# tardis-sn/tardis

Measured on AMD Instinct MI355X. Metric: packets/sec, higher is better.
Workload: dtype f64; 1 GPU; BASELINE configs[2]: 100000000 packets/GPU/step, 20 shells, 500000 lines, macroatom, 0 v-packets, last-interaction tracking on; synthetic opacities (SURVEY 8d, heavy-tailed macro-atom blocks), packets from the device black-body source (T_inner = 10000 K); level_sizes=heavy, packets_per_gpu=100000000, n_shells=20, n_lines=500000, line_interaction_type=macroatom, n_vpackets=0, parallelism=single GPU

## Files before the change

include/tardis_mc.h:

```cpp
#ifndef TARDIS_MC_H
#define TARDIS_MC_H

#include <stdint.h>

#ifdef __cplusplus
extern "C" {
#endif

#define TARDIS_MC_ABI_VERSION 2

enum {
    TARDIS_MC_OK = 0,
    TARDIS_MC_ERR_INVALID_ARGUMENT = -1,
    TARDIS_MC_ERR_HIP = -2,
    TARDIS_MC_ERR_MONTECARLO = -3,
    TARDIS_MC_ERR_MACRO_ATOM = -4,
    TARDIS_MC_ERR_UNSUPPORTED = -5,
    TARDIS_MC_ERR_COMM = -6,
    TARDIS_MC_ERR_STATE = -7
};

enum { TARDIS_MC_LINE_SCATTER = 0, TARDIS_MC_LINE_DOWNBRANCH = 1, TARDIS_MC_LINE_MACROATOM = 2 };

typedef struct TardisMcConfig {
// ... 355 lines not shown
int tardis_mc_streamed_packets(TardisMcContext *ctx, int64_t *out_streamed, int64_t *out_resent);

int tardis_mc_run(TardisMcContext *ctx, const TardisMcPackets *packets, const TardisMcGeometry *geometry,
                  const TardisMcOpacity *opacity, const TardisMcConfig *config, TardisMcResult *result);

#define TARDIS_MC_UNIQUE_ID_BYTES 128
int tardis_mc_comm_get_unique_id(uint8_t out_id[TARDIS_MC_UNIQUE_ID_BYTES]);
int tardis_mc_comm_init(TardisMcContext *ctx, int rank, int world_size,
                        const uint8_t id[TARDIS_MC_UNIQUE_ID_BYTES]);
int tardis_mc_allreduce_estimators(TardisMcContext *ctx);
int tardis_mc_comm_check(TardisMcContext *ctx, int *out_ranks);

int tardis_mc_debug_eval(TardisMcContext *ctx, int op, const double *x, const double *y, double *out, int64_t n);
int tardis_mc_debug_nlte_solve(TardisMcContext *ctx, int64_t n, int64_t n_systems, const double *m, const double *b, double *x, int32_t *status);
int tardis_mc_debug_microbench(TardisMcContext *ctx, int which, int64_t n_doubles, int iters, int blocks, double *out_ms);

#ifdef __cplusplus
}
#endif
#endif
```

tardis_amd/_lib.py:

```python
from __future__ import annotations

import ctypes as C
import os
import subprocess

from . import _abi

_HERE = os.path.dirname(os.path.abspath(__file__))
LIB_PATH = os.environ.get("TARDIS_MC_LIB") or os.path.join(_HERE, "libtardis_mc_hip.so")
_lib = None

_vp, _i, _ll = C.c_void_p, C.c_int, C.c_longlong
SYMBOLS = {
    "tardis_mc_abi_version": (_i, []),
    "tardis_mc_device_count": (_i, []),
    "tardis_mc_create": (_i, [_i, C.POINTER(_vp)]),
    "tardis_mc_destroy": (None, [_vp]),
    "tardis_mc_last_error": (C.c_char_p, [_vp]),
    "tardis_mc_set_option": (_i, [_vp, C.c_char_p, _ll]),
    "tardis_mc_set_geometry": (_i, [_vp, _vp]),
    "tardis_mc_set_opacity": (_i, [_vp, _vp]),
    "tardis_mc_set_config": (_i, [_vp, _vp]),
    "tardis_mc_set_packets": (_i, [_vp, _vp]),
    "tardis_mc_reset_estimators": (_i, [_vp]),
# ... 63 lines not shown
    "tardis_mc_set_nlte_collision_data": (_i, [_vp, _vp]),
    "tardis_mc_check_nlte_collision_data": (_i, [_vp, C.c_int64, _vp, C.c_double, C.c_int64, _vp]),
    "tardis_mc_get_nlte_collision_rates": (_i, [_vp, _vp, _vp]),
    "tardis_mc_get_event_log": (_i, [_vp, _vp]),
    "tardis_mc_get_vpacket_log": (_i, [_vp, _vp]),
    "tardis_mc_stream_results": (_i, [_vp, _vp]),
    "tardis_mc_streamed_packets": (_i, [_vp, C.POINTER(C.c_int64), C.POINTER(C.c_int64)]),
    "tardis_mc_run": (_i, [_vp] * 6),
    "tardis_mc_comm_get_unique_id": (_i, [_vp]),
    "tardis_mc_comm_init": (_i, [_vp, _i, _i, _vp]),
    "tardis_mc_allreduce_estimators": (_i, [_vp]),
    "tardis_mc_comm_check": (_i, [_vp, C.POINTER(_i)]),
    "tardis_mc_debug_eval": (_i, [_vp, _i, _vp, _vp, _vp, C.c_int64]),
    "tardis_mc_debug_nlte_solve": (_i, [_vp, C.c_int64, C.c_int64, _vp, _vp, _vp, _vp]),
    "tardis_mc_debug_microbench": (_i, [_vp, _i, C.c_int64, _i, _i, C.POINTER(C.c_double)]),
}


class EngineUnavailable(RuntimeError):
    """The HIP engine cannot be used (library not built, or no GPU)."""


def build(force: bool = False) -> str:
    cmd = ["make", "-C", os.path.join(_HERE, "csrc")] + (["-B"] if force else [])
    r = subprocess.run(cmd, capture_output=True, text=True)
    if r.returncode != 0:
        raise RuntimeError("building libtardis_mc_hip.so failed:\n" + r.stdout + r.stderr)
    return LIB_PATH


# ... 21 lines not shown
```

tardis_amd/csrc/mc_device.hpp:

```cpp
#pragma once
#include <hip/hip_runtime.h>
#include <stdint.h>
#include "mc_math.hpp"

namespace mc {

constexpr double C_LIGHT = 2.99792458e10;
constexpr double CLOSE_LINE_THRESHOLD = 1e-14;
constexpr double MISS_DISTANCE = 1e99;

enum : int { IT_BOUNDARY = 1, IT_LINE = 2, IT_ESCATTERING = 4 };
enum : int { ST_IN_PROCESS = 0, ST_EMITTED = 1, ST_REABSORBED = 2 };
enum : int { ERR_MONTECARLO = -3, ERR_MACRO_ATOM = -4, ERR_UNSUPPORTED = -5 };

constexpr int MT_N = 624;

template <bool WIDE> struct RowOffset { typedef unsigned type; };
template <> struct RowOffset<true> { typedef unsigned long long type; };
template <bool WIDE> using row_t = typename RowOffset<WIDE>::type;
template <bool WIDE> __host__ __device__ __forceinline__ row_t<WIDE> row_of(int shell, int len) { return (row_t<WIDE>)(unsigned)shell * (row_t<WIDE>)(unsigned)len; }

struct __attribute__((aligned(8))) LineVisitRecord {
    double c_e, c_jb;
    unsigned idx0;
// ... 96 lines not shown
    int n_shells, n_lines, n_trans;
    int line_interaction_type, disable_line_scattering, debug_flags, n_est_copies;
    double t_exp, sigma_thomson;
    double tc, rcp_tc;
    const double *r_inner, *r_outer, *nu_line, *tau_t, *n_e, *prob_t;
    const int2 *line_block;
    const int4 *trans_rec;
    const double *cum_t, *trans_nu;
    const unsigned short *cum16;
    const struct WalkRec *rec16;
    const int2 *quad_info;
    unsigned cum16_stride;
    const unsigned *hot_sec;
    const int2 *blk_tab;
    unsigned hot_stride;
    double *jblue_t, *edot_t;
    long long est_copy_stride;
    unsigned long long *next_packet;
    long long n_vpackets;
    double survival_probability, tau_russian, spawn_start, spawn_end, grid0, grid_last, delta_nu;
    double *vhist;
    const int *bucket_first;
    int bucket_shift, bucket_n;
    long long bucket_kmin;
    const double *tau_pfx, *tau_rowsum;
    const double *nt_t;
    unsigned nt_stride;
};

struct Packet {
// ... 215 lines not shown
```

tardis_amd/csrc/propagate_plan.hpp:

```cpp
#pragma once

#include "../../include/tardis_mc.h"

namespace plan {

constexpr int DBG_WALK_LANE_FP64 = 128;
constexpr int DBG_WALK_GROUP_FP64 = 8192;
constexpr int DBG_LONG_INSTANTIATIONS = 1048576;
constexpr int DBG_NO_SCREENING = 33554432;
constexpr int DBG_SKIP_FALLBACK = 536870912;
constexpr int DBG_WAVE_COUNTERS = 1 | 2 | 4 | 16 | 32 | 16384 | 32768 | 65536 | 131072 | 524288 | 2097152 | 4194304 | 8388608 | 16777216 | 134217728 | 268435456;
constexpr int DBG_FP64_WALKS = DBG_WALK_LANE_FP64 | DBG_WALK_GROUP_FP64;
constexpr int DBG_WAVE_CROSS_CHECK = DBG_FP64_WALKS | DBG_LONG_INSTANTIATIONS | DBG_WAVE_COUNTERS;

struct PlanInput {
    int n_shells, n_lines, n_trans;
    long long n_packets;
    long long number_of_vpackets;
    double survival_probability;
    int enable_full_relativity, line_interaction_type;
    bool lines_sorted, prob_negative, have_walk_tables;
    int variant, table_offsets, vpacket_screening;
    long long vpk_wave_min_packets;
    bool track_full;
    int debug_flags;
    bool pfx_valid, pfx_negative;
// ... 95 lines not shown
```

tardis_amd/csrc/propagate_wave.hpp:

```cpp
#pragma once
#include "mc_device.hpp"
#include "propagate_group.hpp"
#include "estimator_log.hpp"
#include "walk_tables.hpp"
#include "event_log.hpp"
#include "mt_generation.hpp"
#include "sweep_skip.hpp"

namespace mc {

constexpr int WV_STATE_STRIDE = 624;
constexpr int WV_RING = 8, WV_RING_VPK = 16;
enum : int { WS_NEED_PACKET = 0, WS_NEED_TRACE = 1, WS_SWEEP = 2, WS_DONE = 3, WS_WALK = 4, WS_VOLLEY = 5, WS_VCARRY = 6 };
constexpr int RES_PENDING = -1;
constexpr int WV_DBG_FLAGS = 1 | 2 | 4 | 16 | 32 | 16384 | 32768 | 65536 | 131072 | 524288 | 2097152 | 4194304 | 8388608 | 16777216 | 134217728 | 268435456;
constexpr int WV_RESERVE = 32;

struct WaveShared {
    double nu[64], rcp_nu[64], comov_nu[64], chi[64], rcp_chi[64], tau_event[64], d_cont0[64];
    double d_boundary[64];
    int res_info[64], res_line[64];
    unsigned rng_a[64], rng_b[64];
    int cursor[64], rowfast[64];
    int queue[64];
};
constexpr size_t WAVE_SHARED_LS_BYTES = sizeof(WaveShared) - 3 * 64 * sizeof(int);
static_assert(offsetof(WaveShared, queue) + sizeof(int) * 64 == sizeof(WaveShared) && offsetof(WaveShared, cursor) + 3 * 64 * sizeof(int) == sizeof(WaveShared),
              "cursor | rowfast | queue are the last 768 bytes: the lane-sweep instantiations leave them out, the pooled volleys' item list lies over them");
struct WaveSharedFull {
    double r[64], mu[64];
// ... 76 lines not shown
    LaneSave *save;
    WaveSave *wsave;
    int resume;
    int drain_split;
    unsigned *suspended;
    VolleyRequest *vq_req;
    unsigned *vq_items;
    unsigned *vq_count;
    int log_continue;
    int log_gen;
    double *vq_jsave;
    int rng_complete;
    int sweep_skip;
    unsigned sk_ct_off, sk_pn_off;
    double sk_margin;
};

__global__ void __launch_bounds__(64) late_list_kernel(const LaneSave *__restrict__ save, const WaveSave *__restrict__ wsave, int waves, long long first, long long end,
                                                       unsigned *__restrict__ late, unsigned *__restrict__ late_count, unsigned capacity)
{
    const int w = blockIdx.x, lane = threadIdx.x;
    if (w >= waves) return;
    const WaveSave ws = wsave[w];
    if (ws.done) return;
    const LaneSave &v = save[(size_t)w * 64 + lane];
    const bool live = v.state != WS_NEED_PACKET && v.state != WS_DONE && (long long)v.pkt >= first && (long long)v.pkt < end;
    const long long r0 = ws.res_next > first ? ws.res_next : first, r1 = ws.res_end < end ? ws.res_end : end;
    const int n_res = r1 > r0 ? (int)(r1 - r0) : 0;
    const unsigned long long lm = __ballot(live);
    const unsigned n_live = (unsigned)__popcll(lm);
// ... 583 lines not shown
    int ev_chunk = -1;
    unsigned ev_used = 0;
    bool ev_row = false;
    int ev_type = 0, ev_shell = 0, ev_after = 0, ev_absorb = -1, ev_emit = -1;
    double ev_bnu = 0.0, ev_bmu = 0.0, ev_be = 0.0;
    bool exhausted = false;
    long long res_next = 0, res_end = 0;
    int q_head = 0, q_tail = 0;
    unsigned log_used = 0;
    int log_chunk = -1;
    bool logged_any = false;
    unsigned long long visits = 0;
    constexpr bool DBG = XWALK;
    unsigned dbg_rounds = 0;
    unsigned long long dbg_vsteps = 0, dbg_vbusy = 0;
    unsigned dbg_walk = 0;
    bool s_active = false, s_fast = false;
    int s_line = 0;
    row_t<WIDE> s_row = 0;
    double s_tau = 0.0, s_tau_event = 0.0, s_kp = 0.0, s_xb = 0.0;
    int2 pre_blk = make_int2(0, 0);

    auto draw = [&]() {
        const double v = ring[r_head * 64 + lane];
        r_head = (r_head + 1) & (RING - 1);
        --r_cnt;
        ++draws;
        return v;
    };
    auto refill = [&](unsigned long long need, uint32_t *seeded_states) {
// ... 295 lines not shown
                    emit = p.next_line_id;
                    if (P.line_interaction_type != 0) {
                        const int2 blk = LS ? pre_blk : gload(P.line_block + (unsigned)p.next_line_id);
                        mb0 = blk.x; mb1 = blk.y;
                        in_macro = true;
                    }
                }
            }
        }
        TMC_SEC(1)
        if (P.cum16) {
            const int walk_cut = (DBG && (H.debug_flags & 16777216)) ? H.walk_min_active : (H.walk_min_active * __popcll(__ballot(state != WS_DONE))) >> 6;
            bool redo = false;
            double event = 0.0;
            if (resumed && mb1 >= 0 && (mb1 & WALK_REDO)) { redo = true; mb1 &= ~WALK_REDO; event = sh.tau_event[lane]; }
            for (int round = 0;; ++round) {
                const unsigned long long walking = __ballot(in_macro);
                if (!walking) break;
                if ((!VPK || !LS) && round > 0 && __popcll(walking) <= walk_cut && __ballot(!in_macro && state != WS_DONE)) break;
                refill(__ballot(in_macro && !redo && r_cnt < 1), seeded_states);
                unsigned x = 0;
                if (in_macro) {
                    if (!redo) event = draw();
                    x = (unsigned)(event * 65536.0);
                }
                const bool hot = in_macro && mb1 < 0, cold = in_macro && mb1 >= 0;
                int q_lo = 0, q_hi = cold ? (mb1 + 7) >> 3 : 0;
                const MC_G unsigned short *__restrict__ blk = glob(P.cum16) + ((size_t)p.shell * P.cum16_stride + (unsigned)(cold ? mb0 : 0));
                if (DBG && (H.debug_flags & 16384)) dbg_walk += (unsigned)__popcll(__ballot(cold && mb1 > 8 * WALK_WINDOW_QUADS));
                while (__ballot(cold && mb1 > 8 * WALK_WINDOW_QUADS && q_hi - q_lo > WALK_WINDOW_QUADS - 1)) {
                    if (cold && mb1 > 8 * WALK_WINDOW_QUADS && q_hi - q_lo > WALK_WINDOW_QUADS - 1) {
                        const int qm = q_lo + ((q_hi - q_lo) >> 1);
                        const unsigned v = blk[8 * qm + 7];
                        if (v < x) q_lo = qm + 1; else q_hi = qm;
                    }
                }
                int sel = -1;
                bool exact = false;
                int nxt = 0;
                unsigned nxt_arg = 0;
                if (in_macro) {
                    const int nq = hot ? 4 : min(WALK_WINDOW_QUADS, ((mb1 + 7) >> 3) - q_lo);
                    typedef unsigned u4v __attribute__((ext_vector_type(4)));
                    const MC_G u4v *__restrict__ wp = hot ? reinterpret_cast<const MC_G u4v *>(glob(P.hot_sec) + ((size_t)p.shell * (size_t)P.hot_stride + (size_t)(unsigned)mb0 * 16))
                                                          : reinterpret_cast<const MC_G u4v *>(blk + 8 * q_lo);
                    uint4 w0 = make_uint4(0, 0, 0, 0), w1 = w0, w2 = w0, w3 = w0;
                    if (nq > 0) { const u4v t = wp[0]; w0 = make_uint4(t.x, t.y, t.z, t.w); }
                    if (nq > 1) { const u4v t = wp[1]; w1 = make_uint4(t.x, t.y, t.z, t.w); }
                    if (nq > 2) { const u4v t = wp[2]; w2 = make_uint4(t.x, t.y, t.z, t.w); }
                    if (nq > 3) { const u4v t = wp[3]; w3 = make_uint4(t.x, t.y, t.z, t.w); }
                    if (hot) {
                        const unsigned lo2[3] = {w0.x, w0.y, w0.z}, hi2[3] = {w0.w, w1.x, w1.y}, k2[3] = {w3.x, w3.y, w3.z};
                        const unsigned dw[HOT_ENTRIES] = {w1.z, w1.w, w2.x, w2.y, w2.z, w2.w};
                        bool hit = false;
                        unsigned d = 0, k16 = 0;
#pragma unroll
                        for (int e = 0; e < HOT_ENTRIES; ++e) {
                            const unsigned sh16 = 16u * (unsigned)(e & 1);
                            const unsigned l = (lo2[e >> 1] >> sh16) & 0xffffu, h = (hi2[e >> 1] >> sh16) & 0xffffu;
                            if (x >= l && x < h) { hit = true; d = dw[e]; k16 = (k2[e >> 1] >> sh16) & 0xffffu; }
                        }
                        if (hit) {
                            macro += k16 + 1u;
                            if (d & WALK_EMIT) { emit = (int)(d & 0x7fffffffu); in_macro = false; nxt = 3; }
                            else if (d & WALK_HOT_DEST) mb0 = (int)(d & 0x3fffffffu);
                            else { nxt = 2; nxt_arg = d; }
                        } else { redo = true; nxt = 2; nxt_arg = (unsigned)mb0; }
                    } else {
                        const unsigned xx = x | (x << 16);
                        unsigned less = 0, gt = 0;
                        if (nq > 0) walk_count_quad(w0, xx, less, gt);
                        if (nq > 1) walk_count_quad(w1, xx, less, gt);
                        if (nq > 2) walk_count_quad(w2, xx, less, gt);
                        if (nq > 3) walk_count_quad(w3, xx, less, gt);
                        const int n_less = (int)((less & 0xffffu) + (less >> 16)), n_gt = (int)((gt & 0xffffu) + (gt >> 16));
                        int k = 8 * q_lo + n_less;
                        if (8 * nq - n_gt - n_less > 0) {
                            exact = true;
                            const MC_G double *__restrict__ cum = glob(P.cum_t) + (size_t)p.shell * (size_t)P.n_trans;
                            for (; k < mb1; ++k) {
                                const unsigned v = blk[k];
                                if (v > x) break;
                                const int2 qi = gload(P.quad_info + ((unsigned)(mb0 + k) >> 3));
                                if (cum[(unsigned)(qi.x + (k & 7))] > event) break;
                            }
                        }
                        if (k < mb1) sel = k;
                        macro += (unsigned)(sel >= 0 ? sel + 1 : mb1);
                        redo = false;
                        if (sel < 0) { err = ERR_MACRO_ATOM; in_macro = false; }
                        else nxt = 1;
                    }
                }
                if (DBG && (H.debug_flags & 32768)) dbg_walk += (unsigned)__popcll(__ballot(exact));
                if (DBG && (H.debug_flags & 65536)) dbg_walk += (unsigned)__popcll(__ballot(hot && !redo));
                if (DBG && (H.debug_flags & 131072)) dbg_walk += (unsigned)__popcll(__ballot(hot && redo));
                if (nxt == 1) {
                    const WalkRec rec = gload(P.rec16 + (unsigned)(mb0 + sel));
                    if (rec.b & WALK_EMIT) {
                        emit = (int)rec.a;
                        emit_nu_walk = rec.nu;
                        in_macro = false;
                        if (rec.b & WALK_UNSUPPORTED) err = ERR_UNSUPPORTED;
                    } else { mb0 = (int)rec.a; mb1 = (rec.b & WALK_HOT) ? -1 : (int)rec.b; }
                } else if (nxt == 2) {
                    const int2 bt = gload(P.blk_tab + nxt_arg);
                    mb0 = bt.x; mb1 = bt.y;
                } else if (nxt == 3)
                    emit_nu_walk = (NT != 0 && emit < L - 1) ? glob(P.nt_t)[2u * ((unsigned)p.shell * P.nt_stride + (unsigned)emit)]
                                                             : glob(P.nu_line)[(unsigned)emit];
            }
// ... 867 lines not shown
        }
        if (!keep) {
            if (cn[0]) gatomic_add_u64(&C->counters[0], cn[0]);
            if (cn[1]) gatomic_add_u64(&C->counters[1], cn[1]);
            if (cn[2]) gatomic_add_u64(&C->counters[2], cn[2]);
            if (cn[3]) gatomic_add_u64(&C->counters[5], cn[3]);
            if (VPK) {
                if (cn[4]) gatomic_add_u64(&C->counters[3], cn[4]);
                if (cn[5]) gatomic_add_u64(&C->counters[4], cn[5]);
                if (cn[6]) gatomic_add_u64(&C->counters[7], cn[6]);
            }
        }
        if (H.debug_flags & 16) gatomic_add_u64(&C->counters[7], (unsigned long long)dbg_rounds);
        if (VPK && (H.debug_flags & 134217728)) gatomic_add_u64(&C->counters[7], dbg_vbusy);
        if (VPK && (H.debug_flags & 268435456)) gatomic_add_u64(&C->counters[7], dbg_vsteps);
        if (H.debug_flags & (16384 | 32768 | 65536 | 131072)) gatomic_add_u64(&C->counters[7], (unsigned long long)dbg_walk);
        if (H.debug_flags & 2097152) gatomic_add_u64(&C->counters[7], dbg_drain_t0 ? wall_clock64() - dbg_drain_t0 : 0ull);
        if (H.debug_flags & 4194304) gatomic_add_u64(&C->counters[7], (unsigned long long)dbg_drain_passes);
        if (H.debug_flags & 8388608) gatomic_add_u64(&C->counters[7], (unsigned long long)dbg_drain_lanes);
        if (H.debug_flags & 32) gatomic_add_u64(&C->counters[7], (unsigned long long)dbg_passes);
#ifdef TMC_SECTION_TIMERS
        if (H.debug_flags & 64) {
            unsigned long long tsel = 0;
#pragma unroll
            for (int i = 0; i < 8; ++i) if (((H.debug_flags >> 8) & 7) == i) tsel = sec_t[i];
            gatomic_add_u64(&C->counters[7], tsel);
        }
#endif
    }
}

// ... 131 lines not shown
```

tardis_amd/csrc/tardis_mc_hip.hip:

```cpp
#include <hip/hip_runtime.h>
#include <dlfcn.h>

#include <algorithm>
#include <chrono>
#include <cstdarg>
#include <cstdio>
#include <cmath>
#include <cstring>
#include <functional>
#include <numeric>
#include <atomic>
#include <mutex>
#include <string>
#include <vector>

#include "../../include/tardis_mc.h"
#include "mc_device.hpp"
#include "propagate_lane.hpp"
#include "event_log.hpp"
#include "propagate_group.hpp"
#include "estimator_log.hpp"
#include "estimator_partition.hpp"
#include "propagate_wave.hpp"
#include "packet_source.hpp"
// ... 155 lines not shown
        long long bucket_kmin = 0;
        bool lines_sorted = true;
        bool prob_negative = false;
        std::vector<int> h_idx[5];
        std::vector<double> h_nu;
        bool h_macro = false;
        void release() { release_buffers(nu_line, tau_t, n_e, prob_t, cum_t, trans_nu, line2level, block_edge, ttype, dest, tline, line_block, trans_rec, bucket_first); }
    } ot;
    struct WalkTables {
        DevBuf cum16, rec16, quad_info, line_block_c;
        DevBuf hot_sec, hot_mass, hot_flag, blk_tab;
        bool have_hot = false;
        long long n_hot_blocks = 0;
        int walk_hot = -1;
        int walk_hot_min_mass = 800, walk_hot_min_mass_long = 400;
        unsigned cum16_stride = 0;
        bool have_walk_tables = false;
        int walk_sector_packing = 1;
        void release() { release_buffers(cum16, rec16, quad_info, line_block_c, hot_sec, hot_mass, hot_flag, blk_tab); }
    } wt;
    struct ScreeningTables {
        DevBuf tau_pfx, tau_rowsum, pfx_flag;
        bool pfx_valid = false, pfx_negative = false;
        int vpacket_screening = -1;
        void release() { release_buffers(tau_pfx, tau_rowsum, pfx_flag); }
    } sc;
    struct SweepTable {
        int sweep_table = -1;
        DevBuf nt_t;
        bool nt_valid = false, nt_negative = false;
// ... 37 lines not shown
    struct EventLog {
        bool track_full = false;
        long long evlog_capacity = 0;
        long long evlog_max_bytes = 16LL << 30;
        DevBuf ev_rows, ev_fill, ev_state, ev_counts, ev_offsets, ev_tiles, ev_cols;
        bool ev_valid = false;
        long long ev_packets = 0, ev_capacity = 0, ev_slots = 0;
        unsigned ev_chunk_rows = 128, ev_n_chunks = 0;
        void release() { release_buffers(ev_rows, ev_fill, ev_state, ev_counts, ev_offsets, ev_tiles, ev_cols); }
    } el;
    struct WaveResources {
        bool walk_min_active_user = false, ls_min_active_user = false;
        int walk_min_active = 8;
        int tracker_defer = 1, last_tracker_defer = -1;
        int rng_complete = 1;
        long long tracker_pack_max_lines = 0;
        int ls_min_active = 8, ls_max_steps = 1 << 30;
        int drain_split = 0;
        int log_tail_packets = 8;
        int log_tail_split = 1;
        int est_accumulate = 3;
        int est_pipeline = 1;
        DevBuf log_part;
        long long log_chunk_records = 0;
        long long log_capacity = 2500000000LL;
        bool log_capacity_user = false;
        hipStream_t stream2 = nullptr;
        hipEvent_t ev_join = nullptr;
        int pass_cus = 0, pass_cus_built = 0;
        hipStream_t stream_prop_m = nullptr, stream_pass_m = nullptr;
// ... 1307 lines not shown
    wc.vp_scratch = ctx->wv.vp_scratch.as<mc::VpResult>();
    wc.vp_park = (vpk && !E.vq_on && ctx->wv.vp_carry_min_active > 0) ? ctx->wv.vp_park.as<mc::VpPark>() : nullptr;
    wc.vp_carry_min_active = ctx->wv.vp_carry_min_active; wc.trk_defer = E.trk_defer;
    wc.save = E.may_suspend ? E.cur_save : nullptr;
    wc.wsave = E.may_suspend ? E.cur_wsave : nullptr;
    wc.resume = epoch > 0 ? 1 : 0;
    wc.drain_split = E.split_armed ? 64 : (E.compact_armed ? ctx->wv.drain_compact : 0);
    wc.suspended = ctx->wv.suspended_dev.as<unsigned>();
    wc.vq_req = E.vq_on ? ctx->wv.vq_req.as<mc::VolleyRequest>() : nullptr;
    wc.vq_items = E.vq_on ? ctx->wv.vq_items.as<unsigned>() : nullptr;
    wc.vq_count = vq ? ctx->wv.vq_count.as<unsigned>() : nullptr;
    wc.vq_jsave = vq ? ctx->wv.vq_jsave.as<double>() : nullptr;
    wc.log_continue = vq ? 1 : 0;
    wc.log_gen = E.log_gen;
    wc.rng_complete = ctx->wv.rng_complete;
    wc.sweep_skip = E.sweep_skip; wc.sk_ct_off = ctx->sw.sk_ct_off; wc.sk_pn_off = ctx->sw.sk_pn_off; wc.sk_margin = ctx->sw.sk_margin;
    HIP_TRY(ctx, store_value(E.st, wc_dev, wc));
    return TARDIS_MC_OK;
}

int launch_second_half(TardisMcContext *ctx, WaveCall &E, int epoch, int waves1, hipStream_t es, mc::WaveCold *wc_dev)
{
    const mc::WaveCold &wc = ctx->wv.wave_cold_host[epoch & 1];
    mc::WaveCold wc2 = wc;
    wc2.seeded_states = wc.seeded_states + (size_t)waves1 * 64 * mc::WV_STATE_STRIDE;
    if (wc.save) wc2.save = wc.save + (size_t)waves1 * 64;
    if (wc.wsave) wc2.wsave = wc.wsave + waves1;
    if (wc.vp_scratch) wc2.vp_scratch = wc.vp_scratch + (size_t)waves1 * 64 * mc::VP_ROUND;
    if (wc.vp_park) wc2.vp_park = wc.vp_park + (size_t)waves1 * 64;
    HIP_TRY(ctx, hipStreamWaitEvent(es, ctx->wv.ev_split[0], 0));
// ... 221 lines not shown
    const bool vpk = call.vpk, full = call.full, vq = call.plan.variant == 4;
    const int cus = call.cus;
    const long long n = ctx->pk.n_packets;
    const mc::DeviceProblem &F = ctx->problem_host;
    if (n >= (1LL << 31)) return fail(ctx, TARDIS_MC_ERR_INVALID_ARGUMENT, "more than 2^31 packets per propagate call");
    WaveChoice w{};
    int rc = choose_wave_kernel(ctx, call, P, w);
    if (rc) return rc;
    if (w.compact_walk) {
        P.cum16 = ctx->wt.cum16.as<unsigned short>(); P.rec16 = ctx->wt.rec16.as<mc::WalkRec>(); P.quad_info = ctx->wt.quad_info.as<int2>();
        P.cum16_stride = ctx->wt.cum16_stride;
        P.line_block = ctx->wt.line_block_c.as<int2>();
        P.hot_sec = ctx->wt.have_hot ? ctx->wt.hot_sec.as<unsigned>() : nullptr;
        P.blk_tab = ctx->wt.blk_tab.as<int2>();
        P.hot_stride = (unsigned)(16u * (unsigned)ctx->n_levels);
    }
    ctx->pg.progress_wave = true;
    const int n_xcd = 8;
    const bool cu_split = ctx->wv.pass_cus > 0 && !vq && ctx->wv.log_sets != 1 && cus == 32 * n_xcd && n >= 30000000LL;
    const int cus_prop = cu_split ? cus - n_xcd * ctx->wv.pass_cus : cus;
    const int waves = (int)std::max<long long>(1, std::min<long long>((n + 63) / 64, (long long)cus_prop * std::min(w.waves_per_cu, w.max_waves_per_cu) * (vq ? ctx->wv.vq_oversubscribe : 1)));
    if (ctx->el.track_full) {
        rc = setup_event_log(ctx, ctx->problem_host, 4LL * waves);
        if (rc) return rc;
    }
    if (ctx->wv.events_host && ctx->wv.ev_events && hipEventQuery(ctx->wv.ev_events) == hipSuccess && ctx->wv.events_host[1] > 0)
        ctx->wv.traces_per_packet = (double)ctx->wv.events_host[0] / (double)ctx->wv.events_host[1];
    if (1.1 * ctx->wv.traces_per_packet > ctx->wv.log_budget_per_packet) ctx->wv.log_budget_per_packet = 1.3 * ctx->wv.traces_per_packet;
    LogSizing s{};
    rc = size_line_log(ctx, call, w, n, waves, cu_split, s);
// ... 309 lines not shown
    else if (n == "blocks_per_cu") ctx->blocks_per_cu = std::max(1, (int)value);
    else if (n == "track_last_interaction") ctx->pk.track = value != 0;
    else if (n == "estimator_copies") { ctx->es.est_copies = std::max(1, std::min(8, (int)value)); ctx->es.est_valid = false; }
    else if (n == "vpacket_log_capacity") { ctx->vl.vlog_capacity = value; ctx->vl.vlog_capacity_user = value > 0; }
    else if (n == "track_full") ctx->el.track_full = value != 0;
    else if (n == "vpacket_last_interaction") ctx->vl.vlog_li = value != 0;
    else if (n == "event_log_capacity") ctx->el.evlog_capacity = std::max<long long>(0, value);
    else if (n == "event_log_max_bytes") ctx->el.evlog_max_bytes = std::max<long long>(1LL << 20, value);
    else if (n == "debug_flags") ctx->debug_flags = (int)value;
    else if (n == "drain_split") ctx->wv.drain_split = value ? 1 : 0;
    else if (n == "drain_compact") ctx->wv.drain_compact = (int)std::max<long long>(0, std::min<long long>(48, value));
    else if (n == "est_one_level") ctx->wv.est_one_level = value ? 1 : 0;
    else if (n == "drain_pack_lanes") ctx->wv.drain_pack_lanes = (int)std::max<long long>(1, std::min<long long>(64, value));
    else if (n == "walk_sector_packing") ctx->wt.walk_sector_packing = value ? 1 : 0;
    else if (n == "walk_hot") ctx->wt.walk_hot = value < 0 ? -1 : (value ? 1 : 0);
    else if (n == "walk_hot_min_mass") ctx->wt.walk_hot_min_mass = (int)std::max<long long>(0, std::min<long long>(value, 1001));
    else if (n == "walk_hot_min_mass_long") ctx->wt.walk_hot_min_mass_long = (int)std::max<long long>(0, std::min<long long>(value, 1001));
    else if (n == "vpacket_screening") ctx->sc.vpacket_screening = value < 0 ? -1 : (value ? 1 : 0);
    else if (n == "waves_per_simd") ctx->waves_per_simd = (int)value;
    else if (n == "lane_sweep_min_active") {
        ctx->wv.ls_min_active_user = value >= 0;
        ctx->wv.ls_min_active = value >= 0 ? (int)std::min<long long>(value, 63) : 8;
    }
    else if (n == "lane_sweep_max_steps") ctx->wv.ls_max_steps = (int)std::max<long long>(1, value);
    else if (n == "vq_oversubscribe") ctx->wv.vq_oversubscribe = (int)std::max<long long>(1, std::min<long long>(value, 64));
    else if (n == "vq_tracer_waves_per_simd") ctx->wv.vq_tracer_waves_per_simd = (int)std::max<long long>(1, std::min<long long>(value, 16));
    else if (n == "vq_min_items") ctx->wv.vq_min_items = value;
    else if (n == "vq_min_active") ctx->wv.vq_min_active = (int)std::max<long long>(0, std::min<long long>(value, 63));
    else if (n == "log_tail_split") ctx->wv.log_tail_split = value ? 1 : 0;
    else if (n == "est_pipeline") ctx->wv.est_pipeline = value ? 1 : 0;
// ... 5 lines not shown
    else if (n == "stream_min_packets") ctx->rs.min_packets = std::max<long long>(64, value);
    else if (n == "sweep_table") ctx->sw.sweep_table = (int)std::max<long long>(-1, std::min<long long>(value, 2));
    else if (n == "table_offsets") ctx->table_offsets = value < 0 ? -1 : (value ? 1 : 0);
    else if (n == "vpk_wide_registers") ctx->vpk_wide_registers = (int)std::max<long long>(0, std::min<long long>(value, 2));
    else if (n == "bucket_lines_permille") ctx->ot.bucket_lines_permille = (int)std::max<long long>(50, std::min<long long>(value, 16000));
    else if (n == "vp_carry_min_active") ctx->wv.vp_carry_min_active = (int)std::max<long long>(0, std::min<long long>(value, 63));
    else if (n == "est_accumulate") ctx->wv.est_accumulate = (int)std::max<long long>(0, std::min<long long>(value, 3));
    else if (n == "log_tail_packets") ctx->wv.log_tail_packets = (int)std::max<long long>(0, std::min<long long>(value, 1000));
    else if (n == "log_chunk_records") ctx->wv.log_chunk_records = value <= 0 ? 0 : std::max<long long>(256, std::min<long long>(value, 1 << 20));
    else if (n == "walk_min_active") {
        ctx->wv.walk_min_active_user = value >= -1;
        ctx->wv.walk_min_active = value >= -1 ? (int)std::min<long long>(value, 63) : 8;
    }
    else if (n == "tracker_defer") ctx->wv.tracker_defer = value ? 1 : 0;
    else if (n == "rng_complete") ctx->wv.rng_complete = value ? 1 : 0;
    else if (n == "sweep_skip") ctx->sw.sweep_skip = (int)std::max<long long>(-1, std::min<long long>(value, 1));
    else if (n == "tracker_pack_max_lines") ctx->wv.tracker_pack_max_lines = std::max<long long>(0, value);
    else if (n == "group_size") ctx->group_size = (value == 4 || value == 8 || value == 16) ? (int)value : 0;
    else if (n == "pipeline_chunks") {}
    else if (n == "log_capacity") { ctx->wv.log_capacity = std::max<long long>(0, value); ctx->wv.log_capacity_user = true; }
    else if (n == "log_sets") ctx->wv.log_sets = (value == 1 || value == 2) ? (int)value : 0;
    else if (n == "source_max_iterations") ctx->sf.max_iterations = std::max<long long>(1, value);
    else if (n == "chunk_packets") ctx->chunk_packets = std::max<long long>(1024, value);
    else if (n == "opacity_update_long_rows") ctx->ou.long_rows = value < 0 ? -1 : value;
    else if (n == "plasma_update_long_rows") ctx->pl.long_rows = value < 0 ? -1 : value;
    else if (n == "mean_opacity_long_bins") ctx->mo.long_bins = value < 0 ? -1 : value;
    else if (n == "plasma_max_iterations") ctx->pl.max_iterations = std::max<long long>(1, value);
    else if (n == "nlte_lds_levels") ctx->nl.lds_levels = value < 0 ? -1 : value;
    else if (n == "nlte_blocked_levels") ctx->nl.blocked_levels = value < 0 ? -1 : value;
    else return fail(ctx, TARDIS_MC_ERR_INVALID_ARGUMENT, "unknown option '%s'", name);
// ... 51 lines not shown
        long long tc = 0;
        for (size_t b = 0; b < n_levels; ++b) {
            const long long len = (edge[b + 1] - edge[b] + 7) / 8 * 8;
            if (ctx->wt.walk_sector_packing && len > 0) {
                const long long in_sector = tc & 31;
                if (in_sector != 0 && (len > 32 || in_sector + len > 32)) tc += 32 - in_sector;
            }
            c0[b] = tc;
            tc += len;
        }
        c0[n_levels] = tc;
        const long long n_quads = tc / 8;
        const unsigned long long stride = ((unsigned long long)tc + 31ull) / 32ull * 32ull + mc::WALK_SLACK;
        if (tc > 0 && stride * S < (1ull << 32) && tc < (1LL << 30)) {
            std::vector<unsigned char> hot(n_levels, 0);
            if (ctx->wt.walk_hot != 0 && n_levels < (size_t)mc::WALK_HOT) {
                const long long nb = (long long)n_levels * (long long)S;
                HIP_TRY(ctx, ctx->wt.hot_sec.ensure((size_t)nb * 64));
                HIP_TRY(ctx, ctx->wt.hot_mass.ensure((size_t)nb * sizeof(unsigned)));
                HIP_TRY(ctx, ctx->wt.hot_flag.ensure(n_levels));
                auto launch_hot = [&](const unsigned char *flags, unsigned *mass) {
                    hipLaunchKernelGGL(mc::walk_hot_kernel, dim3((unsigned)((nb + 255) / 256)), dim3(256), 0, ctx->stream, ctx->ot.cum_t.as<double>(),
                                       ctx->ot.block_edge.as<int>(), ctx->ot.ttype.as<int>(), ctx->ot.dest.as<int>(), ctx->ot.tline.as<int>(), flags,
                                       (int)n_levels, (long long)T, (int)S, ctx->wt.hot_sec.as<unsigned>(), mass);
                    return hipGetLastError();
                };
                HIP_TRY(ctx, launch_hot(nullptr, ctx->wt.hot_mass.as<unsigned>()));
                std::vector<unsigned> mass((size_t)nb);
                HIP_TRY(ctx, hipMemcpyAsync(mass.data(), ctx->wt.hot_mass.p, (size_t)nb * sizeof(unsigned), hipMemcpyDeviceToHost, ctx->stream));
                HIP_TRY(ctx, hipStreamSynchronize(ctx->stream));
                for (size_t b = 0; b < n_levels; ++b) {
                    const long long rows = edge[b + 1] - edge[b];
                    if (rows <= 0) continue;
                    double m = 0.0;
                    for (size_t sh = 0; sh < S; ++sh) m += (double)mass[sh * n_levels + b];
                    m /= 65536.0 * (double)S;
                    const double need = 1e-3 * (double)(rows > 8 * mc::WALK_WINDOW_QUADS ? ctx->wt.walk_hot_min_mass_long : ctx->wt.walk_hot_min_mass);
                    if (ctx->wt.walk_hot == 1 || m >= need) { hot[b] = 1; ctx->wt.n_hot_blocks += 1; }
                }
                if (ctx->wt.n_hot_blocks > 0) {
                    HIP_TRY(ctx, hipMemcpyAsync(ctx->wt.hot_flag.p, hot.data(), n_levels, hipMemcpyHostToDevice, ctx->stream));
                    hipLaunchKernelGGL(mc::walk_hot_flag_kernel, dim3((unsigned)((nb + 255) / 256)), dim3(256), 0, ctx->stream, ctx->wt.hot_flag.as<unsigned char>(), nb,
                                       ctx->wt.hot_sec.as<unsigned>());
                    HIP_TRY(ctx, hipGetLastError());
                    HIP_TRY(ctx, hipStreamSynchronize(ctx->stream));
                    ctx->wt.have_hot = true;
                } else {
                    ctx->wt.hot_sec.release();
                    ctx->wt.hot_flag.release();
                }
                ctx->wt.hot_mass.release();
            }
            {
                std::vector<int> bt(2 * n_levels);
                for (size_t b = 0; b < n_levels; ++b) {
                    bt[2 * b] = (int)c0[b];
                    bt[2 * b + 1] = (int)(edge[b + 1] - edge[b]);
                }
                if ((rc = upload(ctx, ctx->wt.blk_tab, bt.data(), bt.size()))) return rc;
                HIP_TRY(ctx, hipStreamSynchronize(ctx->stream));
            }
            std::vector<int> qi(2 * (size_t)n_quads, 0), lbc(2 * L, 0);
            std::vector<mc::WalkRec> r16((size_t)tc + 1, mc::WalkRec{0u, 0u, 0.0});
            for (size_t b = 0; b < n_levels; ++b) {
                const long long b0 = edge[b], b1 = edge[b + 1];
                for (long long q = c0[b] / 8, k = b0; k < b1; ++q, k += 8) { qi[2 * q] = (int)k; qi[2 * q + 1] = (int)(b1 - k); }
                for (long long k = b0; k < b1; ++k) {
                    const long long c = c0[b] + (k - b0);
                    const int64_t tt = ttype[k];
                    if (tt >= 0) {
                        const int64_t lvl = dest[k];
                        if (hot[lvl]) { r16[c].a = (unsigned)lvl; r16[c].b = mc::WALK_HOT; }
                        else {
                            r16[c].a = (unsigned)c0[lvl];
                            r16[c].b = (unsigned)(edge[lvl + 1] - edge[lvl]);
// ... 2898 lines not shown
    hipLaunchKernelGGL(comm_check_fill_kernel, dim3(1), dim3(64), 0, ctx->stream, cell.as<double>(), (double)(ctx->rank + 1));
    hipError_t e = hipGetLastError();
    int r = e == hipSuccess ? g_rccl.AllReduce(cell.p, cell.p, 1, 8, 0, ctx->comm, ctx->stream) : 0;
    double got = 0.0;
    if (e == hipSuccess && r == 0) e = hipMemcpyAsync(&got, cell.p, sizeof(double), hipMemcpyDeviceToHost, ctx->stream);
    if (e == hipSuccess && r == 0) e = hipStreamSynchronize(ctx->stream);
    HIP_TRY(ctx, e);
    if (r != 0) return fail(ctx, TARDIS_MC_ERR_COMM, "ncclAllReduce failed: %s", g_rccl.GetErrorString ? g_rccl.GetErrorString(r) : "?");
    const double want = 0.5 * (double)ctx->world * (double)(ctx->world + 1);
    if (got != want)
        return fail(ctx, TARDIS_MC_ERR_COMM, "communicator self-check: the sum of (rank + 1) over %d ranks came back as %.17g, not %.17g", ctx->world, got, want);
    *out_ranks = ctx->world;
    return TARDIS_MC_OK;
}

int tardis_mc_debug_eval(TardisMcContext *ctx, int op, const double *x, const double *y, double *out, int64_t n)
{
    if (!ctx || !x || !out || n <= 0) return TARDIS_MC_ERR_INVALID_ARGUMENT;
    HIP_TRY(ctx, hipSetDevice(ctx->device));
    if (op == 100) {
        const long long first = (long long)x[0], count = n / 8;
        if (n % 8 || first < 0 || first + count > ctx->pk.n_packets || !ctx->pk.li_rec.p || ctx->wv.last_tracker_defer < 0)
            return fail(ctx, TARDIS_MC_ERR_STATE, "debug_eval: no tracker records of a wave-kernel call for packets [%lld, %lld)", first, first + count);
        HIP_TRY(ctx, hipStreamSynchronize(ctx->stream));
        HIP_TRY(ctx, hipMemcpy(out, (const char *)ctx->pk.li_rec.p + (size_t)first * 64, (size_t)count * 64, hipMemcpyDeviceToHost));
        return TARDIS_MC_OK;
    }
    ScopedDevBuf dx, dy, dout, scratch;
    size_t nx = (op == 7) ? 1 : (size_t)n;
    HIP_TRY(ctx, dx.ensure(nx * 8));
// ... 87 lines not shown
```

tardis_amd/csrc/walk_tables.hpp:

```cpp
#pragma once
#include <hip/hip_runtime.h>
#include <stdint.h>

namespace mc {

constexpr unsigned WALK_EMIT = 0x80000000u, WALK_UNSUPPORTED = 0x40000000u;
constexpr unsigned WALK_HOT = 0x20000000u;
constexpr unsigned WALK_HOT_DEST = 0x40000000u;
constexpr int WALK_REDO = 0x40000000;
constexpr int HOT_ENTRIES = 6;
struct __attribute__((aligned(16))) WalkRec {
    unsigned a, b;
    double nu;
};
constexpr int WALK_WINDOW_QUADS = 4;
constexpr int WALK_SLACK = 8 * WALK_WINDOW_QUADS;

__global__ void __launch_bounds__(256) walk_cum16_kernel(const double *__restrict__ cum_t, const int2 *__restrict__ quad_info,
                                                          long long n_quads, long long n_trans, int n_shells, unsigned stride,
                                                          unsigned short *__restrict__ cum16)
{
    const long long i = (long long)blockIdx.x * blockDim.x + threadIdx.x;
    if (i >= n_quads * n_shells) return;
    const long long q = i % n_quads;
    const int s = (int)(i / n_quads);
    const int2 info = quad_info[q];
    const double *c = cum_t + (long long)s * n_trans + info.x;
    unsigned v[8];
#pragma unroll
    for (int k = 0; k < 8; ++k) {
        unsigned e = 0xffffu;
// ... 60 lines not shown
                    t0 = kk[e]; kk[e] = nk; nk = t0;
                }
        }
    }
    unsigned total = 0;
#pragma unroll
    for (int e = 0; e < HOT_ENTRIES; ++e) total += wd[e];
    uint4 *out = reinterpret_cast<uint4 *>(hot_sec + ((size_t)s * (size_t)n_blocks + (size_t)b) * 16);
    out[0] = make_uint4(lo[0] | (lo[1] << 16), lo[2] | (lo[3] << 16), lo[4] | (lo[5] << 16), hi[0] | (hi[1] << 16));
    out[1] = make_uint4(hi[2] | (hi[3] << 16), hi[4] | (hi[5] << 16), dw[0], dw[1]);
    out[2] = make_uint4(dw[2], dw[3], dw[4], dw[5]);
    out[3] = make_uint4(kk[0] | (kk[1] << 16), kk[2] | (kk[3] << 16), kk[4] | (kk[5] << 16), total);
    if (mass) mass[(size_t)s * (size_t)n_blocks + (size_t)b] = total;
}

__global__ void __launch_bounds__(256) walk_hot_flag_kernel(const unsigned char *__restrict__ hot_flag, long long n_records, unsigned *__restrict__ hot_sec)
{
    const long long i = (long long)blockIdx.x * blockDim.x + threadIdx.x;
    if (i >= n_records) return;
    unsigned *rec = hot_sec + (size_t)i * 16;
    const unsigned lo3[3] = {rec[0], rec[1], rec[2]}, hi3[3] = {rec[3], rec[4], rec[5]};
#pragma unroll
    for (int e = 0; e < HOT_ENTRIES; ++e) {
        const unsigned sh16 = 16u * (unsigned)(e & 1);
        const unsigned l = (lo3[e >> 1] >> sh16) & 0xffffu, h = (hi3[e >> 1] >> sh16) & 0xffffu;
        const unsigned d = rec[6 + e];
        if (h > l && !(d & WALK_EMIT) && hot_flag[d & 0x3fffffffu]) rec[6 + e] = d | WALK_HOT_DEST;
    }
}

typedef unsigned short walk_u16x2 __attribute__((ext_vector_type(2)));
__device__ __forceinline__ void walk_count(unsigned d, unsigned xx, unsigned &less, unsigned &gt)
{
    const walk_u16x2 dv = __builtin_bit_cast(walk_u16x2, d), xv = __builtin_bit_cast(walk_u16x2, xx);
    const walk_u16x2 one = {1, 1};
    walk_u16x2 l = __builtin_elementwise_sub_sat(xv, dv);
    walk_u16x2 g = __builtin_elementwise_sub_sat(dv, xv);
    l = __builtin_elementwise_min(l, one);
    g = __builtin_elementwise_min(g, one);
    less = __builtin_bit_cast(unsigned, (walk_u16x2)(__builtin_bit_cast(walk_u16x2, less) + l));
    gt = __builtin_bit_cast(unsigned, (walk_u16x2)(__builtin_bit_cast(walk_u16x2, gt) + g));
}
__device__ __forceinline__ void walk_count_quad(const uint4 &w, unsigned xx, unsigned &less, unsigned &gt)
// ... 6 lines not shown
```

Baseline: 43.23 million packets/s.

## Pack destination block offsets into hot walk records and add cold-batch walk rounds

```diff
diff --git a/include/tardis_mc.h b/include/tardis_mc.h
--- a/include/tardis_mc.h
+++ b/include/tardis_mc.h
@@ -393,6 +393,7 @@
 int tardis_mc_debug_eval(TardisMcContext *ctx, int op, const double *x, const double *y, double *out, int64_t n);
 int tardis_mc_debug_nlte_solve(TardisMcContext *ctx, int64_t n, int64_t n_systems, const double *m, const double *b, double *x, int32_t *status);
 int tardis_mc_debug_microbench(TardisMcContext *ctx, int which, int64_t n_doubles, int iters, int blocks, double *out_ms);
+int tardis_mc_debug_walk_pack(int64_t c0, int64_t rows, int q_bits, int own, int rows_cap, uint32_t *word, int64_t *c0_back, int64_t *rows_back);
 
 #ifdef __cplusplus
 }
diff --git a/tardis_amd/_lib.py b/tardis_amd/_lib.py
--- a/tardis_amd/_lib.py
+++ b/tardis_amd/_lib.py
@@ -101,6 +101,7 @@
     "tardis_mc_debug_eval": (_i, [_vp, _i, _vp, _vp, _vp, C.c_int64]),
     "tardis_mc_debug_nlte_solve": (_i, [_vp, C.c_int64, C.c_int64, _vp, _vp, _vp, _vp]),
     "tardis_mc_debug_microbench": (_i, [_vp, _i, C.c_int64, _i, _i, C.POINTER(C.c_double)]),
+    "tardis_mc_debug_walk_pack": (_i, [C.c_int64, C.c_int64, _i, _i, _i, C.POINTER(C.c_uint32), C.POINTER(C.c_int64), C.POINTER(C.c_int64)]),
 }
 
 
diff --git a/tardis_amd/csrc/mc_device.hpp b/tardis_amd/csrc/mc_device.hpp
--- a/tardis_amd/csrc/mc_device.hpp
+++ b/tardis_amd/csrc/mc_device.hpp
@@ -134,6 +134,7 @@
     const unsigned *hot_sec;
     const int2 *blk_tab;
     unsigned hot_stride;
+    int walk_q;
     double *jblue_t, *edot_t;
     long long est_copy_stride;
     unsigned long long *next_packet;
diff --git a/tardis_amd/csrc/propagate_plan.hpp b/tardis_amd/csrc/propagate_plan.hpp
--- a/tardis_amd/csrc/propagate_plan.hpp
+++ b/tardis_amd/csrc/propagate_plan.hpp
@@ -9,7 +9,7 @@
 constexpr int DBG_LONG_INSTANTIATIONS = 1048576;
 constexpr int DBG_NO_SCREENING = 33554432;
 constexpr int DBG_SKIP_FALLBACK = 536870912;
-constexpr int DBG_WAVE_COUNTERS = 1 | 2 | 4 | 16 | 32 | 16384 | 32768 | 65536 | 131072 | 524288 | 2097152 | 4194304 | 8388608 | 16777216 | 134217728 | 268435456;
+constexpr int DBG_WAVE_COUNTERS = 1 | 2 | 4 | 16 | 32 | 16384 | 32768 | 65536 | 131072 | 262144 | 524288 | 2097152 | 4194304 | 8388608 | 16777216 | 134217728 | 268435456;
 constexpr int DBG_FP64_WALKS = DBG_WALK_LANE_FP64 | DBG_WALK_GROUP_FP64;
 constexpr int DBG_WAVE_CROSS_CHECK = DBG_FP64_WALKS | DBG_LONG_INSTANTIATIONS | DBG_WAVE_COUNTERS;
 
diff --git a/tardis_amd/csrc/propagate_wave.hpp b/tardis_amd/csrc/propagate_wave.hpp
--- a/tardis_amd/csrc/propagate_wave.hpp
+++ b/tardis_amd/csrc/propagate_wave.hpp
@@ -13,7 +13,7 @@
 constexpr int WV_RING = 8, WV_RING_VPK = 16;
 enum : int { WS_NEED_PACKET = 0, WS_NEED_TRACE = 1, WS_SWEEP = 2, WS_DONE = 3, WS_WALK = 4, WS_VOLLEY = 5, WS_VCARRY = 6 };
 constexpr int RES_PENDING = -1;
-constexpr int WV_DBG_FLAGS = 1 | 2 | 4 | 16 | 32 | 16384 | 32768 | 65536 | 131072 | 524288 | 2097152 | 4194304 | 8388608 | 16777216 | 134217728 | 268435456;
+constexpr int WV_DBG_FLAGS = 1 | 2 | 4 | 16 | 32 | 16384 | 32768 | 65536 | 131072 | 262144 | 524288 | 2097152 | 4194304 | 8388608 | 16777216 | 134217728 | 268435456;
 constexpr int WV_RESERVE = 32;
 
 struct WaveShared {
@@ -120,6 +120,7 @@
     int sweep_skip;
     unsigned sk_ct_off, sk_pn_off;
     double sk_margin;
+    int walk_cold_batch;
 };
 
 __global__ void __launch_bounds__(64) late_list_kernel(const LaneSave *__restrict__ save, const WaveSave *__restrict__ wsave, int waves, long long first, long long end,
@@ -733,6 +734,7 @@
     constexpr bool DBG = XWALK;
     unsigned dbg_rounds = 0;
     unsigned long long dbg_vsteps = 0, dbg_vbusy = 0;
+    unsigned dbg_walk_hi = 0;
     unsigned dbg_walk = 0;
     bool s_active = false, s_fast = false;
     int s_line = 0;
@@ -1058,17 +1060,33 @@
             bool redo = false;
             double event = 0.0;
             if (resumed && mb1 >= 0 && (mb1 & WALK_REDO)) { redo = true; mb1 &= ~WALK_REDO; event = sh.tau_event[lane]; }
+            const int cold_k = (LS && !VPK) ? W->walk_cold_batch : 0;
+            unsigned long long moved = 0;
+            bool last_round = false;
             for (int round = 0;; ++round) {
                 const unsigned long long walking = __ballot(in_macro);
-                if (!walking) break;
-                if ((!VPK || !LS) && round > 0 && __popcll(walking) <= walk_cut && __ballot(!in_macro && state != WS_DONE)) break;
-                refill(__ballot(in_macro && !redo && r_cnt < 1), seeded_states);
+                if (!walking || last_round) break;
+                const bool cut = (!VPK || !LS) && round > 0 && __popcll(walking) <= walk_cut && __ballot(!in_macro && state != WS_DONE);
+                bool act = in_macro;
+                if (cold_k > 0) {
+                    if (cut) {
+                        if (!(walking & ~moved)) break;
+                        act = in_macro && !((moved >> lane) & 1ull);
+                        last_round = true;
+                    } else {
+                        const unsigned long long cold_w = __ballot(in_macro && mb1 >= 0);
+                        const bool cold_round = cold_w == walking || __popcll(cold_w) >= cold_k;
+                        act = in_macro && ((mb1 >= 0) == cold_round);
+                    }
+                    moved |= __ballot(act);
+                } else if (cut) break;
+                refill(__ballot(act && !redo && r_cnt < 1), seeded_states);
                 unsigned x = 0;
-                if (in_macro) {
+                if (act) {
                     if (!redo) event = draw();
                     x = (unsigned)(event * 65536.0);
                 }
-                const bool hot = in_macro && mb1 < 0, cold = in_macro && mb1 >= 0;
+                const bool hot = act && mb1 < 0, cold = act && mb1 >= 0;
                 int q_lo = 0, q_hi = cold ? (mb1 + 7) >> 3 : 0;
                 const MC_G unsigned short *__restrict__ blk = glob(P.cum16) + ((size_t)p.shell * P.cum16_stride + (unsigned)(cold ? mb0 : 0));
                 if (DBG && (H.debug_flags & 16384)) dbg_walk += (unsigned)__popcll(__ballot(cold && mb1 > 8 * WALK_WINDOW_QUADS));
@@ -1083,7 +1101,8 @@
                 bool exact = false;
                 int nxt = 0;
                 unsigned nxt_arg = 0;
-                if (in_macro) {
+                bool packed_dest = false;
+                if (act) {
                     const int nq = hot ? 4 : min(WALK_WINDOW_QUADS, ((mb1 + 7) >> 3) - q_lo);
                     typedef unsigned u4v __attribute__((ext_vector_type(4)));
                     const MC_G u4v *__restrict__ wp = hot ? reinterpret_cast<const MC_G u4v *>(glob(P.hot_sec) + ((size_t)p.shell * (size_t)P.hot_stride + (size_t)(unsigned)mb0 * 16))
@@ -1108,8 +1127,13 @@
                             macro += k16 + 1u;
                             if (d & WALK_EMIT) { emit = (int)(d & 0x7fffffffu); in_macro = false; nxt = 3; }
                             else if (d & WALK_HOT_DEST) mb0 = (int)(d & 0x3fffffffu);
-                            else { nxt = 2; nxt_arg = d; }
-                        } else { redo = true; nxt = 2; nxt_arg = (unsigned)mb0; }
+                            else if (d & WALK_DEST_BLOCK) { nxt = 2; nxt_arg = d & (WALK_DEST_BLOCK - 1u); }
+                            else { walk_unpack(d, P.walk_q, mb0, mb1); packed_dest = true; }
+                        } else {
+                            redo = true;
+                            if (w3.w) walk_unpack(w3.w, P.walk_q, mb0, mb1);
+                            else { nxt = 2; nxt_arg = (unsigned)mb0; }
+                        }
                     } else {
                         const unsigned xx = x | (x << 16);
                         unsigned less = 0, gt = 0;
@@ -1139,6 +1163,10 @@
                 if (DBG && (H.debug_flags & 32768)) dbg_walk += (unsigned)__popcll(__ballot(exact));
                 if (DBG && (H.debug_flags & 65536)) dbg_walk += (unsigned)__popcll(__ballot(hot && !redo));
                 if (DBG && (H.debug_flags & 131072)) dbg_walk += (unsigned)__popcll(__ballot(hot && redo));
+                if (DBG && (H.debug_flags & 262144)) {
+                    dbg_walk += (unsigned)__popcll(__ballot(packed_dest));
+                    dbg_walk_hi += (unsigned)__popcll(__ballot(nxt == 2));
+                }
                 if (nxt == 1) {
                     const WalkRec rec = gload(P.rec16 + (unsigned)(mb0 + sel));
                     if (rec.b & WALK_EMIT) {
@@ -2036,7 +2064,7 @@
         if (H.debug_flags & 16) gatomic_add_u64(&C->counters[7], (unsigned long long)dbg_rounds);
         if (VPK && (H.debug_flags & 134217728)) gatomic_add_u64(&C->counters[7], dbg_vbusy);
         if (VPK && (H.debug_flags & 268435456)) gatomic_add_u64(&C->counters[7], dbg_vsteps);
-        if (H.debug_flags & (16384 | 32768 | 65536 | 131072)) gatomic_add_u64(&C->counters[7], (unsigned long long)dbg_walk);
+        if (H.debug_flags & (16384 | 32768 | 65536 | 131072 | 262144)) gatomic_add_u64(&C->counters[7], (unsigned long long)dbg_walk | ((unsigned long long)dbg_walk_hi << 32));
         if (H.debug_flags & 2097152) gatomic_add_u64(&C->counters[7], dbg_drain_t0 ? wall_clock64() - dbg_drain_t0 : 0ull);
         if (H.debug_flags & 4194304) gatomic_add_u64(&C->counters[7], (unsigned long long)dbg_drain_passes);
         if (H.debug_flags & 8388608) gatomic_add_u64(&C->counters[7], (unsigned long long)dbg_drain_lanes);
diff --git a/tardis_amd/csrc/tardis_mc_hip.hip b/tardis_amd/csrc/tardis_mc_hip.hip
--- a/tardis_amd/csrc/tardis_mc_hip.hip
+++ b/tardis_amd/csrc/tardis_mc_hip.hip
@@ -193,6 +193,8 @@
         long long n_hot_blocks = 0;
         int walk_hot = -1;
         int walk_hot_min_mass = 800, walk_hot_min_mass_long = 400;
+        int pack_q_bits = 1;
+        int walk_pack_rows_bits = 0;
         unsigned cum16_stride = 0;
         bool have_walk_tables = false;
         int walk_sector_packing = 1;
@@ -260,6 +262,7 @@
         int walk_min_active = 8;
         int tracker_defer = 1, last_tracker_defer = -1;
         int rng_complete = 1;
+        int walk_cold_batch = 0;
         long long tracker_pack_max_lines = 0;
         int ls_min_active = 8, ls_max_steps = 1 << 30;
         int drain_split = 0;
@@ -1597,6 +1600,7 @@
     wc.log_continue = vq ? 1 : 0;
     wc.log_gen = E.log_gen;
     wc.rng_complete = ctx->wv.rng_complete;
+    wc.walk_cold_batch = ctx->wv.walk_cold_batch;
     wc.sweep_skip = E.sweep_skip; wc.sk_ct_off = ctx->sw.sk_ct_off; wc.sk_pn_off = ctx->sw.sk_pn_off; wc.sk_margin = ctx->sw.sk_margin;
     HIP_TRY(ctx, store_value(E.st, wc_dev, wc));
     return TARDIS_MC_OK;
@@ -1848,6 +1852,7 @@
         P.hot_sec = ctx->wt.have_hot ? ctx->wt.hot_sec.as<unsigned>() : nullptr;
         P.blk_tab = ctx->wt.blk_tab.as<int2>();
         P.hot_stride = (unsigned)(16u * (unsigned)ctx->n_levels);
+        P.walk_q = ctx->wt.pack_q_bits;
     }
     ctx->pg.progress_wave = true;
     const int n_xcd = 8;
@@ -2187,6 +2192,7 @@
     else if (n == "drain_pack_lanes") ctx->wv.drain_pack_lanes = (int)std::max<long long>(1, std::min<long long>(64, value));
     else if (n == "walk_sector_packing") ctx->wt.walk_sector_packing = value ? 1 : 0;
     else if (n == "walk_hot") ctx->wt.walk_hot = value < 0 ? -1 : (value ? 1 : 0);
+    else if (n == "walk_pack_rows_bits") ctx->wt.walk_pack_rows_bits = (int)std::max<long long>(0, std::min<long long>(value, 31));
     else if (n == "walk_hot_min_mass") ctx->wt.walk_hot_min_mass = (int)std::max<long long>(0, std::min<long long>(value, 1001));
     else if (n == "walk_hot_min_mass_long") ctx->wt.walk_hot_min_mass_long = (int)std::max<long long>(0, std::min<long long>(value, 1001));
     else if (n == "vpacket_screening") ctx->sc.vpacket_screening = value < 0 ? -1 : (value ? 1 : 0);
@@ -2222,6 +2228,7 @@
     }
     else if (n == "tracker_defer") ctx->wv.tracker_defer = value ? 1 : 0;
     else if (n == "rng_complete") ctx->wv.rng_complete = value ? 1 : 0;
+    else if (n == "walk_cold_batch") ctx->wv.walk_cold_batch = (int)std::max<long long>(0, std::min<long long>(value, 64));
     else if (n == "sweep_skip") ctx->sw.sweep_skip = (int)std::max<long long>(-1, std::min<long long>(value, 1));
     else if (n == "tracker_pack_max_lines") ctx->wv.tracker_pack_max_lines = std::max<long long>(0, value);
     else if (n == "group_size") ctx->group_size = (value == 4 || value == 8 || value == 16) ? (int)value : 0;
@@ -2303,6 +2310,16 @@
         const unsigned long long stride = ((unsigned long long)tc + 31ull) / 32ull * 32ull + mc::WALK_SLACK;
         if (tc > 0 && stride * S < (1ull << 32) && tc < (1LL << 30)) {
             std::vector<unsigned char> hot(n_levels, 0);
+            {
+                std::vector<int> bt(2 * n_levels);
+                for (size_t b = 0; b < n_levels; ++b) {
+                    bt[2 * b] = (int)c0[b];
+                    bt[2 * b + 1] = (int)(edge[b + 1] - edge[b]);
+                }
+                if ((rc = upload(ctx, ctx->wt.blk_tab, bt.data(), bt.size()))) return rc;
+                HIP_TRY(ctx, hipStreamSynchronize(ctx->stream));
+            }
+            ctx->wt.pack_q_bits = mc::walk_pack_quad_bits(tc);
             if (ctx->wt.walk_hot != 0 && n_levels < (size_t)mc::WALK_HOT) {
                 const long long nb = (long long)n_levels * (long long)S;
                 HIP_TRY(ctx, ctx->wt.hot_sec.ensure((size_t)nb * 64));
@@ -2329,7 +2346,8 @@
                 }
                 if (ctx->wt.n_hot_blocks > 0) {
                     HIP_TRY(ctx, hipMemcpyAsync(ctx->wt.hot_flag.p, hot.data(), n_levels, hipMemcpyHostToDevice, ctx->stream));
-                    hipLaunchKernelGGL(mc::walk_hot_flag_kernel, dim3((unsigned)((nb + 255) / 256)), dim3(256), 0, ctx->stream, ctx->wt.hot_flag.as<unsigned char>(), nb,
+                    hipLaunchKernelGGL(mc::walk_hot_flag_kernel, dim3((unsigned)((nb + 255) / 256)), dim3(256), 0, ctx->stream, ctx->wt.hot_flag.as<unsigned char>(),
+                                       ctx->wt.blk_tab.as<int2>(), ctx->wt.pack_q_bits, ctx->wt.walk_pack_rows_bits, (int)n_levels, nb,
                                        ctx->wt.hot_sec.as<unsigned>());
                     HIP_TRY(ctx, hipGetLastError());
                     HIP_TRY(ctx, hipStreamSynchronize(ctx->stream));
@@ -2339,15 +2357,6 @@
                     ctx->wt.hot_flag.release();
                 }
                 ctx->wt.hot_mass.release();
-            }
-            {
-                std::vector<int> bt(2 * n_levels);
-                for (size_t b = 0; b < n_levels; ++b) {
-                    bt[2 * b] = (int)c0[b];
-                    bt[2 * b + 1] = (int)(edge[b + 1] - edge[b]);
-                }
-                if ((rc = upload(ctx, ctx->wt.blk_tab, bt.data(), bt.size()))) return rc;
-                HIP_TRY(ctx, hipStreamSynchronize(ctx->stream));
             }
             std::vector<int> qi(2 * (size_t)n_quads, 0), lbc(2 * L, 0);
             std::vector<mc::WalkRec> r16((size_t)tc + 1, mc::WalkRec{0u, 0u, 0.0});
@@ -5276,6 +5285,19 @@
     return TARDIS_MC_OK;
 }
 
+int tardis_mc_debug_walk_pack(int64_t c0, int64_t rows, int q_bits, int own, int rows_cap, uint32_t *word, int64_t *c0_back, int64_t *rows_back)
+{
+    if (!word || !c0_back || !rows_back || q_bits < 1 || q_bits > 29 || rows_cap < 0) return TARDIS_MC_ERR_INVALID_ARGUMENT;
+    *word = 0; *c0_back = -1; *rows_back = -1;
+    if (c0 < 0 || rows < 0 || c0 > 0x7fffffffLL || rows > 0x7fffffffLL) return 0;
+    unsigned w = 0;
+    if (!mc::walk_pack((int)c0, (int)rows, q_bits, own ? mc::WALK_PACK_OWN_BITS : mc::WALK_PACK_DEST_BITS, rows_cap, w)) return 0;
+    int c = 0, r = 0;
+    mc::walk_unpack(w, q_bits, c, r);
+    *word = w; *c0_back = c; *rows_back = r;
+    return 1;
+}
+
 int tardis_mc_debug_eval(TardisMcContext *ctx, int op, const double *x, const double *y, double *out, int64_t n)
 {
     if (!ctx || !x || !out || n <= 0) return TARDIS_MC_ERR_INVALID_ARGUMENT;
diff --git a/tardis_amd/csrc/walk_tables.hpp b/tardis_amd/csrc/walk_tables.hpp
--- a/tardis_amd/csrc/walk_tables.hpp
+++ b/tardis_amd/csrc/walk_tables.hpp
@@ -15,6 +15,39 @@
 };
 constexpr int WALK_WINDOW_QUADS = 4;
 constexpr int WALK_SLACK = 8 * WALK_WINDOW_QUADS;
+
+constexpr unsigned WALK_DEST_BLOCK = 0x20000000u;
+constexpr int WALK_PACK_DEST_BITS = 29, WALK_PACK_OWN_BITS = 32;
+__host__ __device__ inline int walk_pack_quad_bits(long long compact_total)
+{
+    int q = 1;
+    while (q < 29 && (compact_total >> 3) >> q) ++q;
+    return q;
+}
+__host__ __device__ inline bool walk_pack(int c0, int rows, int q_bits, int bits, int rows_cap, unsigned &word)
+{
+    int rb = bits - q_bits;
+    if (rows_cap > 0 && rows_cap < rb) rb = rows_cap;
+    word = 0;
+    if (rb <= 0 || c0 < 0 || rows < 0 || (c0 & 7)) return false;
+    const unsigned long long q = (unsigned long long)((unsigned)c0 >> 3), r = (unsigned long long)(unsigned)rows;
+    if ((q >> q_bits) || (r >> rb)) return false;
+    const unsigned w = (unsigned)(q | (r << q_bits));
+    if (bits == WALK_PACK_OWN_BITS && w == 0) return false;
+    word = w;
+    return true;
+}
+__host__ __device__ inline void walk_unpack(unsigned word, int q_bits, int &c0, int &rows)
+{
+    c0 = (int)((word & ((1u << q_bits) - 1u)) << 3);
+    rows = (int)(word >> q_bits);
+}
+__host__ __device__ inline unsigned walk_dest_word(unsigned lvl, bool lvl_is_hot, int2 bt, int q_bits, int rows_cap)
+{
+    if (lvl_is_hot) return lvl | WALK_HOT_DEST;
+    unsigned word;
+    return walk_pack(bt.x, bt.y, q_bits, WALK_PACK_DEST_BITS, rows_cap, word) ? word : (lvl | WALK_DEST_BLOCK);
+}
 
 __global__ void __launch_bounds__(256) walk_cum16_kernel(const double *__restrict__ cum_t, const int2 *__restrict__ quad_info,
                                                           long long n_quads, long long n_trans, int n_shells, unsigned stride,
@@ -105,7 +138,8 @@
     if (mass) mass[(size_t)s * (size_t)n_blocks + (size_t)b] = total;
 }
 
-__global__ void __launch_bounds__(256) walk_hot_flag_kernel(const unsigned char *__restrict__ hot_flag, long long n_records, unsigned *__restrict__ hot_sec)
+__global__ void __launch_bounds__(256) walk_hot_flag_kernel(const unsigned char *__restrict__ hot_flag, const int2 *__restrict__ blk_tab, int q_bits, int rows_cap,
+                                                             int n_blocks, long long n_records, unsigned *__restrict__ hot_sec)
 {
     const long long i = (long long)blockIdx.x * blockDim.x + threadIdx.x;
     if (i >= n_records) return;
@@ -116,8 +150,13 @@
         const unsigned sh16 = 16u * (unsigned)(e & 1);
         const unsigned l = (lo3[e >> 1] >> sh16) & 0xffffu, h = (hi3[e >> 1] >> sh16) & 0xffffu;
         const unsigned d = rec[6 + e];
-        if (h > l && !(d & WALK_EMIT) && hot_flag[d & 0x3fffffffu]) rec[6 + e] = d | WALK_HOT_DEST;
+        if (h <= l || (d & WALK_EMIT)) continue;
+        rec[6 + e] = walk_dest_word(d & 0x3fffffffu, hot_flag[d & 0x3fffffffu] != 0, blk_tab[d & 0x3fffffffu], q_bits, rows_cap);
     }
+    const int2 own = blk_tab[(int)(i % n_blocks)];
+    unsigned word;
+    walk_pack(own.x, own.y, q_bits, WALK_PACK_OWN_BITS, rows_cap, word);
+    rec[15] = word;
 }
 
 typedef unsigned short walk_u16x2 __attribute__((ext_vector_type(2)));
```

After: 42.95 million packets/s. Within noise of the previous version (-0.6%).
